# NinV/Background-Debiased-Video-CIL

Hardware: AMD Instinct MI355X
Metric: clips/sec fwd+bwd TSM-R50 8x224^2 bs32/GPU (higher is better)
Workload: dtype f32; 1 GPU; TSM-ResNet50 fwd+bwd+SGD step, synthetic 32x8x3x224x224 clips per GPU, 101 classes, SimpleLinear+CrossEntropyLoss, dropout 0.5, random-init weights; fp32 tensors, accumulators and results; conv products: fp32 via 3xbf16 split, 6 MFMA products, fp32 accumulate (dropped terms <= 2^-24 relative); conv_arith=bf16x3, clips_per_gpu=32, global_batch=32, parallelism=dp1

## Files before the change

background-debiased-video-cil_amd/_lib.py:

```python
from __future__ import annotations

import ctypes
import os
from ctypes import POINTER, Structure, c_char_p, c_float, c_int, c_int32, c_int64, c_size_t, c_uint16, c_uint64, c_void_p

_HERE = os.path.dirname(os.path.abspath(__file__))
_OVERRIDE = os.environ.get('BDVCIL_LIB_PATH')
LIB_PATH = _OVERRIDE or os.path.join(_HERE, 'csrc', 'libbdvcil_hip.so')
ABI_VERSION = 32

_lib = None


class ConvGeom(Structure):
    _fields_ = [(n, c_int32) for n in
                ('N', 'H', 'W', 'Cin', 'Ho', 'Wo', 'Cout', 'R', 'S', 'stride', 'pad', 'T', 'fold', 'pad_w', 'Rt', 'st_t', 'act_dtype')]

    def key(self):
        return tuple(getattr(self, n) for n, _ in self._fields_)


P = c_void_p
_F3 = c_float * 3

# ... 74 lines not shown
    'bdv_avgpool_fwd': (c_int, [P, P, c_int, c_int, c_int, c_int, P]),
    'bdv_avgpool_bwd': (c_int, [P, P, c_int, c_int, c_int, c_int, P]),
    'bdv_bgmix_normalize_u8': (c_int, [P, P, c_int, P, c_float, _F3, _F3, _F3, P, P, c_int, c_int, c_int, c_int, P]),
    'bdv_bg_resize_crop_u8': (c_int, [P, c_int, c_int, c_int, c_int, c_int, P, P, c_int, c_int, P, P]),
    'bdv_resize_linear_u8': (c_int, [P, c_int, c_int, c_int, P, c_int, P, P, c_int, c_int, P]),
    'bdv_jpeg_parse': (c_int, [P, c_size_t, POINTER(JpegInfo)]),
    'bdv_jpeg_entropy_decode': (c_int, [P, c_size_t, POINTER(JpegInfo), P]),
    'bdv_jpeg_entropy_decode_batch': (c_int, [P, P, c_int, POINTER(JpegInfo), P, P, c_int]),
    'bdv_jpeg_workspace_bytes': (c_size_t, [POINTER(JpegInfo), c_int]),
    'bdv_jpeg_reconstruct_u8': (c_int, [P, P, POINTER(JpegInfo), c_int, P, c_size_t, P, P]),
    'bdv_temporal_median_u8': (c_int, [P, c_int64, P, P, P, P, c_int, c_int, c_int, P, P]),
    'bdv_jpeg_encode_info': (c_int, [c_int, c_int, c_int, POINTER(JpegInfo)]),
    'bdv_jpeg_forward_u8': (c_int, [P, c_int, c_int, c_int, c_int, P, P]),
    'bdv_jpeg_encode_bound': (c_size_t, [c_int, c_int]),
    'bdv_jpeg_entropy_encode': (c_int, [P, c_int, c_int, c_int, P, c_size_t, P]),
    'bdv_jpeg_entropy_encode_batch': (c_int, [P, c_int, c_int, c_int, c_int, P, c_size_t, P, c_int]),
    'bdv_crop_normalize_u8': (c_int, [P, P, c_int, c_int, c_int, _F3, _F3, P, P, c_int, c_int, c_int, c_int, P]),
    'bdv_actor_cut_mix_u8': (c_int, [P, c_int, c_int, c_int, P, c_int, c_int, c_int, P, P, c_int64, c_int, c_int, c_int, c_int, _F3, _F3, P,
                                     c_int, P, P]),
    'bdv_lsc_fwd': (c_int, [P, P, P, P, P, P, c_int, c_int, c_int, c_int, P]),
    'bdv_lsc_bwd': (c_int, [P, P, P, P, P, P, P, P, c_float, P, c_int, c_int, c_int, c_int, P]),
    'bdv_linear_fwd': (c_int, [P, P, P, P, c_int, c_int, c_int, P]),
    'bdv_linear_bwd': (c_int, [P, P, P, P, P, P, c_float, c_int, c_int, c_int, P]),
    'bdv_consensus_fwd': (c_int, [P, P, c_int, c_int, c_int, P]),
    'bdv_consensus_bwd': (c_int, [P, P, c_int, c_int, c_int, P]),
    'bdv_dropout': (c_int, [P, P, c_int64, c_float, c_uint64, P]),
    'bdv_lsc_loss': (c_int, [P, P, P, c_float, c_int, P, P, P, P, c_int, c_int, P]),
    'bdv_softce_loss': (c_int, [P, P, P, P, P, c_int, c_int, P]),
    'bdv_icarl_targets': (c_int, [P, P, c_int, P, P, c_int, c_int, P]),
    'bdv_acm_targets': (c_int, [P, P, P, c_float, P, c_int, c_int, P]),
    'bdv_softmax_mean': (c_int, [P, P, c_int, c_int, c_int, c_int, P]),
    'bdv_topk_acc': (c_int, [P, P, P, c_int, c_int, P]),
    'bdv_repr_from_features': (c_int, [P, P, P, c_int, c_int, c_int, c_int, P]),
    'bdv_nme_workspace_bytes': (c_size_t, [c_int, c_int]),
    'bdv_nme_classify': (c_int, [P, P, P, P, c_int, c_int, c_int, c_int, P, c_size_t, P]),
    'bdv_class_means': (c_int, [P, P, P, c_int, c_int, c_int, P]),
    'bdv_herding_workspace_bytes': (c_size_t, [c_int, c_int]),
    'bdv_herding_select': (c_int, [P, c_int, c_int, c_int, c_int, P, P, P, P, c_size_t, P]),
    'bdv_randaug_workspace_bytes': (c_size_t, [c_int, c_int, c_int, c_int]),
    'bdv_randaug_apply': (c_int, [P, P, P, P, c_int, c_int, c_int, c_int, P, c_size_t, P]),
    'bdv_reduce_workspace_bytes': (c_size_t, []),
    'bdv_kd_mse_fwd': (c_int, [P, P, P, c_int64, P, c_size_t, c_int, P]),
    'bdv_kd_mse_bwd': (c_int, [P, P, P, c_float, P, c_int64, c_int, P]),
    'bdv_multi_sqnorm': (c_int, [P, P, c_int, P, P, c_size_t, P]),
    'bdv_clip_coef': (c_int, [P, c_float, c_float, P, P]),
    'bdv_multi_sgd': (c_int, [P, P, P, P, P, P, c_int, c_float, c_float, P, P]),
}


class HipExtensionError(RuntimeError):
    pass


HASHED_SOURCES = ('conv_mfma.hip', 'bn.hip', 'pool_frontend.hip', 'head_loss.hip', 'repr.hip', 'augment.hip', 'optim.hip', 'jpeg.hip',
                  'background.hip', 'actor_cut_mix.hip', 'api_common.cpp', 'common.h', 'resize_linear.h', 'Makefile', '../../include/bdvcil_hip.h')


def source_hash():
    import hashlib
    h = hashlib.sha256()
    base = os.path.join(_HERE, 'csrc')
    for name in HASHED_SOURCES:
        path = os.path.join(base, name)
        if not os.path.exists(path):
            return None
        with open(path, 'rb') as f:
            h.update(f.read())
    return h.hexdigest()


def lib():
    global _lib
    if _lib is None:
        if not os.path.exists(LIB_PATH):
            raise HipExtensionError(
                f'HIP extension not built: {LIB_PATH} is missing. Run `python -c "import __graft_entry__ as g; '
                f'g.build()"` (or `make -C {os.path.dirname(LIB_PATH)}`). There is no CPU fallback.')
        handle = ctypes.CDLL(LIB_PATH)
        for name, (res, args) in SIGNATURES.items():
            fn = getattr(handle, name)
            fn.restype = res
            fn.argtypes = args
        if handle.bdv_abi_version() != ABI_VERSION:
            raise HipExtensionError(f'ABI mismatch: library {handle.bdv_abi_version()} != binding {ABI_VERSION}')
        want, have = source_hash(), handle.bdv_source_hash().decode()
        if want is not None and want != have and not _OVERRIDE:
            raise HipExtensionError(f'stale library: {LIB_PATH} was built from other sources (hash {have[:12]}, in-tree '
                                    f'{want[:12]}). Rebuild: make -C {os.path.dirname(LIB_PATH)}')
        _lib = handle
    return _lib


def check(code: int, what: str = ''):
    if code != 0:
        msg = lib().bdv_last_error()
        raise HipExtensionError(f'{what or "bdvcil_hip"} failed with code {code}: {msg.decode() if msg else ""}')
```

background-debiased-video-cil_amd/csrc/conv_mfma.hip:

```cpp
#include <stdlib.h>
#include "common.h"

#ifdef BDV_STAMPS
__device__ unsigned long long* g_stamp_buf = nullptr;
__device__ int g_stamp_cap = 0;
#define BDV_STAMP(slot)                                                                                                          \
  do {                                                                                                                           \
    if (threadIdx.x == 0 && g_stamp_buf != nullptr && (int)(blockIdx.x + gridDim.x * blockIdx.y) < g_stamp_cap) {                 \
      unsigned long long* q_ = g_stamp_buf + (size_t)(blockIdx.x + gridDim.x * blockIdx.y) * 8;                                  \
      if ((slot) == 4) asm volatile("s_waitcnt vmcnt(0)" ::: "memory");                                                          \
      q_[slot] = __builtin_amdgcn_s_memtime();                                                                                   \
      if ((slot) == 0) { q_[5] = __builtin_amdgcn_s_memrealtime(); q_[7] = __builtin_amdgcn_s_getreg((4 << 0) | (0 << 6) | (31 << 11)); } \
      if ((slot) == 4) q_[6] = __builtin_amdgcn_s_memrealtime();                                                                 \
    }                                                                                                                            \
  } while (0)
#else
#define BDV_STAMP(slot) do { } while (0)
#endif

namespace {

constexpr int BK = 32;

struct Geom {
  int N, H, W, Cin, Ho, Wo, Cout, R, S, stride, pad, pad_w, T, fold;
  int Rt, st_t;
  float rcp_RS, rcp_S;
  int M;
  int Ktot;
  float rcp_HoWo, rcp_Wo;
  int stagger;
};

typedef unsigned int u32x4 __attribute__((ext_vector_type(4)));
constexpr int kOOB = (int)0x80000000;

__device__ __forceinline__ float4 buf_load16(__amdgpu_buffer_rsrc_t rsrc, int voff, int soff) {
  const u32x4 v = __builtin_amdgcn_raw_buffer_load_b128(rsrc, voff, soff, 0);
  return make_float4(__uint_as_float(v.x), __uint_as_float(v.y), __uint_as_float(v.z), __uint_as_float(v.w));
}

__device__ __forceinline__ void buf_store16(__amdgpu_buffer_rsrc_t rsrc, int voff, float4 v) {
  u32x4 d;
  d.x = __float_as_uint(v.x);
  d.y = __float_as_uint(v.y);
  d.z = __float_as_uint(v.z);
  d.w = __float_as_uint(v.w);
  __builtin_amdgcn_raw_buffer_store_b128(d, rsrc, voff, 0, 0);
}

typedef unsigned int u32x2v __attribute__((ext_vector_type(2)));
template <int ES>
__device__ __forceinline__ float4 buf_ld4(__amdgpu_buffer_rsrc_t rsrc, int voff) {
  if constexpr (ES == 4) {
    return buf_load16(rsrc, voff, 0);
  } else {
    const u32x2v v = __builtin_amdgcn_raw_buffer_load_b64(rsrc, voff, 0, 0);
    return bdv_widen_bf16x4(v.x, v.y);
  }
}
template <int ES>
__device__ __forceinline__ void buf_st4(__amdgpu_buffer_rsrc_t rsrc, int voff, float4 v) {
  if constexpr (ES == 4) {
    buf_store16(rsrc, voff, v);
  } else {
    __builtin_amdgcn_raw_buffer_store_b64((u32x2v){bdv_pack_bf16x2(v.x, v.y), bdv_pack_bf16x2(v.z, v.w)}, rsrc, voff, 0, 0);
  }
}

__device__ __forceinline__ void fast_divmod(int m, int d, float rcp, int& q, int& r) {
  q = (int)((float)m * rcp);
  r = m - q * d;
  if (r < 0) {
    r += d;
    --q;
  }
  if (r >= d) {
    r -= d;
    ++q;
  }
}

template <int LDA, int LDB, int TM, int TN, int MS, int NS, bool SWA, bool SWB>
__device__ __forceinline__ void mma_stage(const float* __restrict__ As, const float* __restrict__ Bs,
                                          f32x16 (&acc)[TM][TN], int wm0, int wn0, int lane) {
  const int r = lane & 31, h = lane >> 5;
  const float* apv[SWA ? 8 : 1];
  const float* bpv[SWB ? 8 : 1];
#pragma unroll
  for (int c = 0; c < (SWA ? 8 : 1); ++c) apv[c] = As + h * LDA + wm0 + (r ^ (4 * c));
#pragma unroll
  for (int c = 0; c < (SWB ? 8 : 1); ++c) bpv[c] = Bs + h * LDB + wn0 + (r ^ (4 * c));
  auto ap = [&](int s, int i) { return apv[SWA ? ((s >> 1) & 7) : 0][2 * s * LDA + MS * i]; };
  auto bp = [&](int s, int j) { return bpv[SWB ? ((s >> 1) & 7) : 0][2 * s * LDB + NS * j]; };
  float a[2][TM], b[2][TN];
#pragma unroll
  for (int i = 0; i < TM; ++i) a[0][i] = ap(0, i);
#pragma unroll
  for (int j = 0; j < TN; ++j) b[0][j] = bp(0, j);
#pragma unroll
  for (int s = 0; s < BK / 2; ++s) {
    const int cur = s & 1, nxt = cur ^ 1;
    if (s + 1 < BK / 2) {
#pragma unroll
      for (int i = 0; i < TM; ++i) a[nxt][i] = ap(s + 1, i);
#pragma unroll
      for (int j = 0; j < TN; ++j) b[nxt][j] = bp(s + 1, j);
    }
#pragma unroll
    for (int i = 0; i < TM; ++i)
#pragma unroll
      for (int j = 0; j < TN; ++j)
        acc[i][j] = __builtin_amdgcn_mfma_f32_32x32x2f32(a[cur][i], b[cur][j], acc[i][j], 0, 0, 0);
    __builtin_amdgcn_sched_group_barrier(0x100, TM + TN, 0);
    __builtin_amdgcn_sched_group_barrier(0x008, TM * TN, 0);
  }
}

__device__ __forceinline__ int shift_class(int c, int fold) {
  return (fold > 0) ? (c < fold ? 1 : (c < 2 * fold ? -1 : 0)) : 0;
}

template <int LD, int PASSES>
__device__ __forceinline__ void store_transposed(float* __restrict__ dst, const float4 (&v)[PASSES], int tid) {
  const int row = tid >> 3, kg = tid & 7;
#pragma unroll
  for (int p = 0; p < PASSES; ++p) {
    float* d = dst + (4 * kg) * LD + ((row + 32 * p) ^ (4 * kg));
    d[0] = v[p].x;
    d[LD] = v[p].y;
    d[2 * LD] = v[p].z;
    d[3 * LD] = v[p].w;
  }
}

template <int LD, int COLS, int PASSES>
__device__ __forceinline__ void store_direct(float* __restrict__ dst, const float4 (&v)[PASSES], int tid) {
  constexpr int V = COLS / 4;
#pragma unroll
  for (int p = 0; p < PASSES; ++p) {
    const int idx = tid + 256 * p;
    const int krow = idx / V, c4 = idx - krow * V;
    *reinterpret_cast<float4*>(dst + krow * LD + 4 * c4) = v[p];
  }
}

__device__ __forceinline__ int acc_row(int reg, int lane) { return (reg & 3) + 8 * (reg >> 2) + 4 * (lane >> 5); }

struct Work {
  int dp_tiles, rem_tiles, split;
};

__device__ __forceinline__ int xcd_remap(int b, int n) {
  const int q = n >> 3, r = n & 7, x = b & 7, j = b >> 3;
  return (x < r ? x * (q + 1) : r * (q + 1) + (x - r) * q) + j;
}

struct WorkItem {
  int tile, kb, ke, pslot;
};

__device__ __forceinline__ WorkItem get_work(int b, const Work& wk, int nk) {
  WorkItem it;
  if (b < wk.dp_tiles) {
    it.tile = xcd_remap(b, wk.dp_tiles);
    it.kb = 0;
    it.ke = nk;
    it.pslot = -1;
  } else {
    const int rem = b - wk.dp_tiles;
    const int rt = rem / wk.split, sl = rem - rt * wk.split;
    it.tile = wk.dp_tiles + rt;
    it.kb = (int)(((long long)sl * nk) / wk.split);
    it.ke = (int)(((long long)(sl + 1) * nk) / wk.split);
    it.pslot = wk.split > 1 ? rem : -1;
  }
  return it;
}

template <int TM, int TN, int NT = 256>
__device__ __forceinline__ void store_partial(float* __restrict__ slab, int pslot, const f32x16 (&acc)[TM][TN], int tid) {
  float* base = slab + (size_t)pslot * (TM * TN * 16) * NT + tid;
#pragma unroll
  for (int i = 0; i < TM; ++i)
#pragma unroll
    for (int j = 0; j < TN; ++j)
#pragma unroll
      for (int e = 0; e < 16; ++e) base[(size_t)((i * TN + j) * 16 + e) * NT] = acc[i][j][e];
}

template <int TM, int TN>
__device__ __forceinline__ void zero_acc(f32x16 (&acc)[TM][TN]) {
#pragma unroll
  for (int i = 0; i < TM; ++i)
#pragma unroll
    for (int j = 0; j < TN; ++j)
#pragma unroll
      for (int e = 0; e < 16; ++e) acc[i][j][e] = 0.f;
}

// ... 372 lines not shown
#pragma unroll
  for (int p = 0; p < BP; ++p) b_base[p] = ((nt * BN + arow + 32 * p) * g.Ktot + 4 * kg) * 4;

  const int RS = g.R * g.S;
  int chunk = it.kb / RS, r, s;
  {
    const int tap = it.kb - chunk * RS;
    r = tap / g.S;
    s = tap - r * g.S;
  }

  float4 ra[AP], rb[BP];
  auto load = [&]() {
    const int cls = shift_class(chunk * BK + 4 * kg, g.fold);
    const int koff_a = ((r * g.W + s) * g.Cin + chunk * BK) * 4;
    const int koff_b = ((r * g.S + s) * g.Cin + chunk * BK) * 4;
#pragma unroll
    for (int p = 0; p < AP; ++p) {
      const bool v = (unsigned)(a_hi0[p] + r) < (unsigned)g.H && (unsigned)(a_wi0[p] + s) < (unsigned)g.W &&
                     (unsigned)(a_t[p] + cls) < (unsigned)g.T;
      ra[p] = buf_load16(xr, (a_base[p] + koff_a + cls * frame_bytes) | (v ? 0 : kOOB), 0);
    }
#pragma unroll
    for (int p = 0; p < BP; ++p) rb[p] = buf_load16(wr, b_base[p], koff_b);
    s += 1;
    const int ws_ = (s == g.S) ? 1 : 0;
    s = ws_ ? 0 : s;
    r += ws_;
    const int wr_ = (r == g.R) ? 1 : 0;
    r = wr_ ? 0 : r;
    chunk += wr_;
  };

  f32x16 acc[TM][TN];
  zero_acc<TM, TN>(acc);

  load();
  for (int kt = it.kb; kt < it.ke; ++kt) {
    __syncthreads();
    store_transposed<LDA, AP>(As, ra, tid);
    store_transposed<LDB, BP>(Bs, rb, tid);
    __syncthreads();
    if (kt + 1 < it.ke) load();
    mma_stage<LDA, LDB, TM, TN, 32 * WM, 32 * WN, true, true>(As, Bs, acc, wm0, wn0, lane);
  }

  if (it.pslot >= 0) {
    store_partial<TM, TN>(slab, it.pslot, acc, tid);
    return;
  }
  fprop_epilogue<BM, BN, WM, WN>(acc, smem, y, g, epi, mt, nt, tid);
}

typedef __bf16 bf16x8_t __attribute__((ext_vector_type(8)));
typedef __bf16 bf16x4_t __attribute__((ext_vector_type(4)));
typedef float f32x4_t __attribute__((ext_vector_type(4)));
constexpr int X3_LDK = BK + 8;

typedef __bf16 bf16x2_t __attribute__((ext_vector_type(2)));
typedef float f32x2_t __attribute__((ext_vector_type(2)));
typedef unsigned u32x2_t __attribute__((ext_vector_type(2)));
__device__ __forceinline__ unsigned pack_bf16x2(float a, float b) {
  return __builtin_bit_cast(unsigned, __builtin_convertvector((f32x2_t){a, b}, bf16x2_t));
}
__device__ __forceinline__ u32x2_t bf16_hi_pairs(const float4 v) { return (u32x2_t){pack_bf16x2(v.x, v.y), pack_bf16x2(v.z, v.w)}; }
__device__ __forceinline__ void split3_pairs(const float4 v, u32x2_t& hi, u32x2_t& mid, u32x2_t& lo) {
  const unsigned h0 = pack_bf16x2(v.x, v.y), h1 = pack_bf16x2(v.z, v.w);
  const float rx = v.x - __uint_as_float(h0 << 16), ry = v.y - __uint_as_float(h0 & 0xffff0000u);
  const float rz = v.z - __uint_as_float(h1 << 16), rw = v.w - __uint_as_float(h1 & 0xffff0000u);
  const unsigned m0 = pack_bf16x2(rx, ry), m1 = pack_bf16x2(rz, rw);
  const float sx = rx - __uint_as_float(m0 << 16), sy = ry - __uint_as_float(m0 & 0xffff0000u);
  const float sz = rz - __uint_as_float(m1 << 16), sw = rw - __uint_as_float(m1 & 0xffff0000u);
  hi = (u32x2_t){h0, h1};
  mid = (u32x2_t){m0, m1};
  lo = (u32x2_t){pack_bf16x2(sx, sy), pack_bf16x2(sz, sw)};
}

template <int ROWS, int P>
__device__ __forceinline__ void store_split3(unsigned short* __restrict__ dst, const float4 (&v)[P], int tid) {
  const int arow = tid >> 3, kg = tid & 7;
#pragma unroll
  for (int p = 0; p < P; ++p) {
    u32x2_t hi, mid, lo;
    split3_pairs(v[p], hi, mid, lo);
    unsigned short* q = dst + (arow + 32 * p) * X3_LDK + 4 * kg;
    *reinterpret_cast<u32x2_t*>(q) = hi;
    *reinterpret_cast<u32x2_t*>(q + ROWS * X3_LDK) = mid;
    *reinterpret_cast<u32x2_t*>(q + 2 * ROWS * X3_LDK) = lo;
  }
}

template <int TM, int TN, int MS, int NS, int ROWS_A, int ROWS_B>
__device__ __forceinline__ void mma_stage_x3(const unsigned short* __restrict__ As, const unsigned short* __restrict__ Bs,
                                             f32x16 (&acc)[TM][TN], int wm0, int wn0, int lane) {
  const int r = lane & 31, h = lane >> 5;
#pragma unroll
  for (int s = 0; s < BK / 16; ++s) {
    bf16x8_t a[3][TM], b[3][TN];
#pragma unroll
    for (int p = 0; p < 3; ++p) {
#pragma unroll
      for (int i = 0; i < TM; ++i)
        a[p][i] = *reinterpret_cast<const bf16x8_t*>(As + (p * ROWS_A + wm0 + MS * i + r) * X3_LDK + 16 * s + 8 * h);
#pragma unroll
      for (int j = 0; j < TN; ++j)
        b[p][j] = *reinterpret_cast<const bf16x8_t*>(Bs + (p * ROWS_B + wn0 + NS * j + r) * X3_LDK + 16 * s + 8 * h);
    }
#pragma unroll
    for (int i = 0; i < TM; ++i)
#pragma unroll
      for (int j = 0; j < TN; ++j) {
        acc[i][j] = __builtin_amdgcn_mfma_f32_32x32x16_bf16(a[1][i], b[1][j], acc[i][j], 0, 0, 0);
        acc[i][j] = __builtin_amdgcn_mfma_f32_32x32x16_bf16(a[0][i], b[2][j], acc[i][j], 0, 0, 0);
        acc[i][j] = __builtin_amdgcn_mfma_f32_32x32x16_bf16(a[2][i], b[0][j], acc[i][j], 0, 0, 0);
        acc[i][j] = __builtin_amdgcn_mfma_f32_32x32x16_bf16(a[0][i], b[1][j], acc[i][j], 0, 0, 0);
        acc[i][j] = __builtin_amdgcn_mfma_f32_32x32x16_bf16(a[1][i], b[0][j], acc[i][j], 0, 0, 0);
        acc[i][j] = __builtin_amdgcn_mfma_f32_32x32x16_bf16(a[0][i], b[0][j], acc[i][j], 0, 0, 0);
      }
  }
}

template <int BM, int BN, int WM, int WN, bool BPRE = false>
__global__ __launch_bounds__(256, 2) void conv_fprop_x3_kernel(const float* __restrict__ x, const float* __restrict__ w,
                                                          float* __restrict__ y, Geom g, int NT, Work wk,
                                                          float* __restrict__ slab, FpropEpi epi) {
  constexpr int TM = BM / WM / 32, TN = BN / WN / 32;
  constexpr int AP = BM / 32, BP = BN / 32;
  static_assert(3 * (BM + BN) * X3_LDK * 2 >= WM * 32 * BN * 4, "the epilogue stages a tile pass in the same LDS");
  __shared__ __attribute__((aligned(16))) unsigned short smem16[3 * (BM + BN) * X3_LDK];
// ... 1955 lines not shown
  if (ncols % 256 != 0) return taps > 1 && stride == 1 ? 1 : (small_tiles && taps == 1 && stride == 1 && nk >= 16 ? 4 : -1);
  if (stride == 2 && taps > 1) return 0;
  if (small_tiles && shifted && taps == 1) return 4;
  if (nk <= 8 && ncols >= 1024) return -1;
  if (shifted && taps == 1 && (ncols >= 512 || nk >= 4)) return -1;
  if (ncols == 512 && nk >= 64) return 0;
  return 2;
}

PlPlan plan_pl(int cfg, int M, int ncols, int nk, size_t ws_bytes, bool ksplit_ok) {
  PlPlan p;
  p.cfg = cfg;
  p.est_us = 0.0;
  if (cfg < 0) return p;
  const PlCfg& k = kPlCfg[cfg];
  p.MT = (M + k.BM - 1) / k.BM;
  p.NT = ncols / k.BN;
  p.nk = nk;
  p.seg_bytes = (size_t)k.BM * k.BN * sizeof(float);
  if (ksplit_ok && cfg != 4) {
    p.wk = plan_work_pl(p.MT * p.NT, nk, k.iter_us, p.seg_bytes, ws_bytes, &p.est_us, pl_cfg_round(cfg));
  } else {
    p.wk.dp_tiles = p.MT * p.NT;
    p.wk.rem_tiles = 0;
    p.wk.split = 1;
    p.est_us = (double)((p.MT * p.NT + 255) / 256) * nk * k.iter_us;
  }
  return p;
}

constexpr bool r1_planes_enabled() { return true; }

bool c4_x3_enabled() {
  static const bool on = getenv("BDVCIL_C4_X3") == nullptr || atoi(getenv("BDVCIL_C4_X3")) != 0;
  return on;
}

int pl_fprop_cfg(const bdv_conv_geom* g, int pieces = 3) {
  if (g->Cin % BK != 0) return -1;
  return pl_pick(false, g->Cout, g->R * g->S * g->Cin / BK, g->R * g->S, g->stride, pieces);
}
int pl_dgrad_cfg(const bdv_conv_geom* g, int pieces = 3) {
  if (g->Cout % BK != 0) return -1;
  return pl_pick(true, g->Cin, g->R * g->S * g->Cout / BK, g->R * g->S, g->stride, pieces, g->fold > 0);
}
bool pl_fprop_ok(const bdv_conv_geom* g, int pieces = 3) { return pl_fprop_cfg(g, pieces) >= 0; }
int pl_fprop_cfg_pre(const bdv_conv_geom* g) {
  if (g->Cin % BK != 0 || g->Cout % 64 != 0) return -1;
  const int cfg = pl_fprop_cfg(g, 3);
  if (cfg >= 0) return cfg;
  return g->Cout % 256 == 0 ? 0 : g->Cout % 128 == 0 ? 1 : 3;
}
bool pl_dgrad_ok(const bdv_conv_geom* g, int pieces = 3) { return pl_dgrad_cfg(g, pieces) >= 0; }


struct WgradPlan {
  bool small;
  bool c4;
  int MTw, NTw, splits, kt_per_split;
};

WgradPlan plan_wgrad(const bdv_conv_geom* g) {
  static const int W = getenv("BDVCIL_WGRAD_W") ? atoi(getenv("BDVCIL_WGRAD_W")) : 768;
  WgradPlan p;
  p.c4 = (g->Cin % BK) != 0;
  p.small = p.c4 || (g->Cout % 128) != 0 || (g->Cin % 128) != 0;
  const int bm = p.small ? 64 : 128, bn = p.small ? 64 : 128;
  const int ktot = g->R * g->S * g->Cin;
  p.MTw = g->Cout / bm;
  p.NTw = p.c4 ? (ktot + bn - 1) / bn : g->R * g->S * (g->Cin / bn);
  const int64_t M = (int64_t)g->N * g->Ho * g->Wo;
  const int nkt = (int)((M + BK - 1) / BK);
  const int tiles = p.MTw * p.NTw;
  int best_s = 1;
  double best_cost = 1e30;
  const double dw_bytes = (double)g->Cout * ktot * 4.0;
  const int Wk = p.small ? 2 * W : W;
  for (int k = 1; k <= 4; ++k) {
    int sp = (int)(((long long)k * Wk) / tiles);
    if (sp < 1) sp = 1;
    if (sp > 1024) sp = 1024;
    while (sp > 1 && (nkt + sp - 1) / sp < 4) --sp;
    const int per = (nkt + sp - 1) / sp;
    const double rounds = (double)(((long long)tiles * sp + Wk - 1) / Wk);
    const double t_iter = 1.7 * 3.0 * (p.small ? 0.25 : 1.0);
    const double cost = rounds * per * t_iter + 4.0 + sp * dw_bytes / 4.0e6;
    if (cost < best_cost) {
      best_cost = cost;
      best_s = sp;
    }
  }
  const int per = (nkt + best_s - 1) / best_s;
  p.kt_per_split = per;
  p.splits = (nkt + per - 1) / per;
  return p;
}

bool wgrad_two_stage() {
  const char* e = getenv("BDVCIL_WGRAD_2STAGE");
  return e == nullptr || atoi(e) != 0;
}

int pl_wgrad_form(const bdv_conv_geom* g) {
  static const bool small_on = getenv("BDVCIL_PL_WGRAD64") == nullptr || atoi(getenv("BDVCIL_PL_WGRAD64")) != 0;
  const int RS = g->R * g->S;
  if (g->Cin % 128 == 0 && g->Cout % 128 == 0) return 0;
// ... 227 lines not shown
  BDV_LAUNCH_CHECK("bdv_conv_dgrad");
  if (p.wk.split > 1) {
    const dim3 fg(p.wk.rem_tiles);
    if (p.wide)
      hipLaunchKernelGGL((conv_dgrad_fixup_kernel<128, 128, 2, 2>), fg, dim3(256), 0, s, (const float*)slab, dx, add_src, add_mask_src, g, p.NT, p.wk, stat);
    else
      hipLaunchKernelGGL((conv_dgrad_fixup_kernel<128, 64, 2, 2>), fg, dim3(256), 0, s, (const float*)slab, dx, add_src, add_mask_src, g, p.NT, p.wk, stat);
    BDV_LAUNCH_CHECK("bdv_conv_dgrad(fixup)");
  }
  return BDV_OK;
}
}

extern "C" int bdv_conv_dgrad(const float* dy, const float* w, float* dx, const float* add_src,
                              const uint32_t* add_mask_src, const bdv_conv_geom* gg, const bdv_bn_stat_fuse* bn_stat,
                              void* workspace, size_t workspace_bytes, void* stream) {
  return conv_dgrad_impl(dy, w, nullptr, dx, add_src, add_mask_src, gg, bn_stat, workspace, workspace_bytes, stream);
}

extern "C" int bdv_conv_dgrad_x3(const float* dy, const float* w, const float* w_t, float* dx, const float* add_src,
                                 const uint32_t* add_mask_src, const bdv_conv_geom* gg, const bdv_bn_stat_fuse* bn_stat,
                                 void* workspace, size_t workspace_bytes, void* stream) {
  BDV_REQUIRE(w_t != nullptr, "bdv_conv_dgrad_x3: w_t is null");
  return conv_dgrad_impl(dy, w, w_t, dx, add_src, add_mask_src, gg, bn_stat, workspace, workspace_bytes, stream);
}

extern "C" size_t bdv_conv_weight_planes_bytes(const bdv_conv_geom* gg) {
  if (check_geom(gg, "bdv_conv_weight_planes_bytes")) return 0;
  return (size_t)3 * gg->Cout * gg->R * gg->S * gg->Cin * sizeof(unsigned short);
}

#ifdef BDV_STAMPS
extern "C" int bdv_debug_set_stamps(void* buf, int cap_workgroups) {
  unsigned long long* p = (unsigned long long*)buf;
  if (hipMemcpyToSymbol(HIP_SYMBOL(g_stamp_buf), &p, sizeof(p)) != hipSuccess) return -1;
  if (hipMemcpyToSymbol(HIP_SYMBOL(g_stamp_cap), &cap_workgroups, sizeof(int)) != hipSuccess) return -1;
  return 0;
}
#endif

extern "C" int bdv_conv_debug_force_tile(int cfg) {
  BDV_REQUIRE(cfg >= -1 && cfg <= kNumPlCfg, "bdv_conv_debug_force_tile: cfg %d (-1 automatic, 0 = 128x256, 1 = 256x128, 2 = 256x256, 3 = 256x64, 4 = 64x128 (dgrad), 5 = 128x128 (four waves), 6 = none)", cfg);
  g_pl_tile_forced = cfg;
  return BDV_OK;
}

extern "C" int bdv_conv_kernel_name(const bdv_conv_geom* gg, int kind, int arith, char* out, size_t n) {
  if (int e = check_geom(gg, "bdv_conv_kernel_name")) return e;
  BDV_REQUIRE(out && n > 0 && kind >= 0 && kind <= 2, "bdv_conv_kernel_name: bad argument");
  const bool c4 = gg->Cin % BK != 0;
  const int pieces = arith == 2 ? 1 : arith == 3 ? 2 : 3;
  if (kind == 0) {
    const int cfg = arith ? pl_fprop_cfg(gg, pieces) : -1;
    if (cfg >= 0) {
      snprintf(out, n, "conv_fprop_pl_kernel<%d, %d, %d, %d, %d, %d>", kPlCfg[cfg].BM, kPlCfg[cfg].BN, pl_cfg_wm(cfg), pl_cfg_wn(cfg), kPlCfg[cfg].nbuf, pieces);
    } else if (c4) {
      snprintf(out, n, "conv_fprop_c4_%skernel<128, %d, 2, 2>", arith && c4_x3_enabled() ? "x3_" : "", gg->Cout % 128 == 0 ? 128 : 64);
    } else if (gg->Cout % 128 == 0 && arith) {
      snprintf(out, n, "conv_fprop_x3_kernel<128, 128, 2, 2, %s>", r1_planes_enabled() ? "true" : "false");
    } else {
      snprintf(out, n, "conv_fprop_kernel<128, %d, 2, 2>", gg->Cout % 128 == 0 ? 128 : 64);
    }
  } else if (kind == 1) {
    const int cfg = arith ? pl_dgrad_cfg(gg, pieces) : -1;
    if (cfg >= 0) {
      snprintf(out, n, "conv_dgrad_pl_kernel<%d, %d, %d, %d, %d, %d>", kPlCfg[cfg].BM, kPlCfg[cfg].BN, pl_cfg_wm(cfg), pl_cfg_wn(cfg), kPlCfg[cfg].nbuf, pieces);
    } else if (gg->Cin % 128 == 0 && arith) {
      snprintf(out, n, "conv_dgrad_x3_kernel<128, 128, 2, 2, %s>", r1_planes_enabled() ? "true" : "false");
    } else {
      snprintf(out, n, "conv_dgrad_kernel<128, %d, 2, 2>", gg->Cin % 128 == 0 ? 128 : 64);
    }
  } else {
    if (arith && pl_wgrad_ok(gg)) {
      const WgradPlPlan p = plan_wgrad_pl(gg);
      snprintf(out, n, "conv_wgrad_pl_kernel<%d, %d", p.BM, p.BN);
    } else {
      const WgradPlan p = plan_wgrad(gg);
      snprintf(out, n, "conv_wgrad_kernel<%d, %d, 2, 2", p.small ? 64 : 128, p.small ? 64 : 128);
    }
  }
  return BDV_OK;
}

extern "C" int bdv_conv_uses_planes(const bdv_conv_geom* gg, int kind, int pieces) {
  if (check_geom(gg, "bdv_conv_uses_planes")) return 0;
  if (kind == 0) return pl_fprop_ok(gg, pieces) || (pieces >= 2 && r1_planes_enabled() && gg->Cin % BK == 0 && gg->Cout % 128 == 0) ? 1 : 0;
  if (kind == 1) return pl_dgrad_ok(gg, pieces) || (pieces >= 2 && r1_planes_enabled() && gg->Cout % BK == 0 && gg->Cin % 128 == 0) ? 1 : 0;
  return 0;
}

extern "C" int bdv_conv_fprop_pl_stat_rows(const bdv_conv_geom* gg, int pieces) {
  if (check_geom(gg, "bdv_conv_fprop_pl_stat_rows")) return 0;
  if (!pl_fprop_ok(gg, pieces)) return bdv_conv_fprop_stat_rows(gg);
  const PlPlan p = plan_pl(pl_fprop_cfg(gg, pieces), gg->N * gg->Ho * gg->Wo, gg->Cout, gg->R * gg->S * gg->Cin / BK, kMaxSplitWorkspace, true);
  return p.cfg >= 0 ? p.MT : 0;
}

extern "C" int bdv_conv_fprop_pre_stat_rows(const bdv_conv_geom* gg) {
  if (check_geom(gg, "bdv_conv_fprop_pre_stat_rows")) return 0;
  const int cfg = pl_fprop_cfg_pre(gg);
  if (cfg < 0) return 0;
  const PlPlan p = plan_pl(cfg, gg->N * gg->Ho * gg->Wo, gg->Cout, gg->R * gg->S * gg->Cin / BK, kMaxSplitWorkspace, true);
  return p.MT;
}

extern "C" int bdv_conv_dgrad_pl_stat_rows(const bdv_conv_geom* gg, int pieces) {
  if (check_geom(gg, "bdv_conv_dgrad_pl_stat_rows")) return 0;
  if (!pl_dgrad_ok(gg, pieces)) return bdv_conv_dgrad_stat_rows(gg);
  const int st = gg->stride;
  const int Mc0 = gg->N * ((gg->H + st - 1) / st) * ((gg->W + st - 1) / st);
  const PlPlan p = plan_pl(pl_dgrad_cfg(gg, pieces), st == 1 ? gg->N * gg->H * gg->W : Mc0, gg->Cin, gg->R * gg->S * gg->Cout / BK,
                           kMaxSplitWorkspace, st == 1);
  return p.cfg >= 0 ? st * st * p.MT : 0;
}

extern "C" int bdv_conv_split_weights(const float* w, const bdv_conv_geom* gg, void* planes_fprop, void* planes_dgrad, void* stream) {
  if (int e = check_geom(gg, "bdv_conv_split_weights")) return e;
  BDV_REQUIRE(w && (planes_fprop || planes_dgrad), "bdv_conv_split_weights: null pointer");
  BDV_REQUIRE(gg->Cin % 32 == 0 && gg->Cout % 32 == 0, "bdv_conv_split_weights: Cin=%d and Cout=%d must be multiples of 32", gg->Cin, gg->Cout);
  BDV_REQUIRE(bdv_aligned16(w) && bdv_aligned16(planes_fprop) && bdv_aligned16(planes_dgrad), "bdv_conv_split_weights: alignment");
  const dim3 grid(gg->Cin / 32, gg->Cout / 32, gg->R * gg->S);
  hipLaunchKernelGGL(split_weights_kernel, grid, dim3(256), 0, (hipStream_t)stream, w, (unsigned short*)planes_fprop,
                     (unsigned short*)planes_dgrad, gg->Cout, gg->R * gg->S, gg->Cin);
  BDV_LAUNCH_CHECK("bdv_conv_split_weights");
  return BDV_OK;
}

extern "C" int bdv_conv_fprop_pre_ok(const bdv_conv_geom* gg) {
  if (check_geom(gg, "bdv_conv_fprop_pre_ok")) return 0;
  return pl_fprop_cfg_pre(gg) >= 0 && gg->fold == 0 ? 1 : 0;
}

extern "C" int bdv_conv_fprop_pl(const void* x, const float* w, const void* planes_fprop, void* y, const bdv_conv_geom* gg,
                                 float* bn_partial, const bdv_conv_affine* affine, void* workspace, size_t workspace_bytes,
                                 int pieces, const float* pre_scale, const float* pre_shift, void* stream) {
  if (int e = check_geom(gg, "bdv_conv_fprop_pl")) return e;
  BDV_REQUIRE(pieces >= 1 && pieces <= 3, "bdv_conv_fprop_pl: pieces = %d (3, 2 or 1)", pieces);
  const bool pre = pre_scale != nullptr;
  const bool h16 = gg->act_dtype == BDV_ACT_BF16;
  BDV_REQUIRE_ACT(gg->act_dtype, "bdv_conv_fprop_pl");
  if (h16)
    BDV_REQUIRE(pieces == 1 && !pre && planes_fprop != nullptr && pl_fprop_ok(gg, 1),
                "bdv_conv_fprop_pl: bf16 activation storage needs pieces = 1, the weight planes, Cin %% 32 == 0 and Cout %% 64 == 0 (Cin=%d Cout=%d)", gg->Cin, gg->Cout);
  if (pre) {
    BDV_REQUIRE(pre_shift != nullptr && planes_fprop != nullptr && pieces == 3 && gg->fold == 0 && pl_fprop_cfg_pre(gg) >= 0,
                "bdv_conv_fprop_pl: a producer BatchNorm in the loader needs the plane kernels (pieces 3, no temporal shift, Cin %% 32 == 0)");
    BDV_REQUIRE(bdv_aligned16(pre_scale) && bdv_aligned16(pre_shift), "bdv_conv_fprop_pl: pre_scale / pre_shift must be 16-byte aligned");
  }
  if (!pre && (planes_fprop == nullptr || !pl_fprop_ok(gg, pieces)))
    return conv_fprop_impl((const float*)x, w, (float*)y, gg, bn_partial, affine, workspace, workspace_bytes, stream, true,
                           gg->Cin % BK == 0 && r1_planes_enabled() ? planes_fprop : nullptr);
  BDV_REQUIRE(x && y, "bdv_conv_fprop_pl: null pointer");
  FpropEpi epi = {bn_partial, 0, nullptr, nullptr, nullptr, 0, pre_scale, pre_shift};
  if (affine != nullptr) {
    BDV_REQUIRE(bn_partial == nullptr, "bdv_conv_fprop_pl: batch statistics and the folded eval-mode BatchNorm exclude each other");
    BDV_REQUIRE(affine->scale && affine->shift, "bdv_conv_fprop_pl: null pointer in bdv_conv_affine");
    BDV_REQUIRE(bdv_aligned16(affine->scale) && bdv_aligned16(affine->shift) && bdv_aligned16(affine->residual),
                "bdv_conv_fprop_pl: bdv_conv_affine pointers must be 16-byte aligned");
    epi.scale = affine->scale;
    epi.shift = affine->shift;
    epi.res = affine->residual;
    epi.relu = affine->relu;
  }
  BDV_REQUIRE(bdv_aligned16(x) && bdv_aligned16(planes_fprop) && bdv_aligned16(y) && bdv_aligned16(workspace),
              "bdv_conv_fprop_pl: pointers must be 16-byte aligned");
  Geom g = make_geom(gg);
  g.M = g.N * g.Ho * g.Wo;
  g.Ktot = g.Rt * g.R * g.S * g.Cin;
  BDV_REQUIRE((int64_t)3 * g.Cout * g.Ktot * 2 < (1ll << 31), "bdv_conv_fprop_pl: weight planes exceed 2^31 bytes");
  hipStream_t s = (hipStream_t)stream;
  const PlPlan p = plan_pl(pre ? pl_fprop_cfg_pre(gg) : pl_fprop_cfg(gg, pieces), g.M, g.Cout, g.Ktot / BK, workspace ? (workspace_bytes < kMaxSplitWorkspace ? workspace_bytes : kMaxSplitWorkspace) : 0, !h16);
  BDV_REQUIRE(p.cfg >= 0, "bdv_conv_fprop_pl: no tile configuration for Cout=%d", g.Cout);
  const int blocks = p.wk.dp_tiles + p.wk.rem_tiles * p.wk.split;
  epi.MT = p.MT;
  float* slab = (float*)workspace;
  const unsigned short* wp = (const unsigned short*)planes_fprop;
  if (debug_plan())
    fprintf(stderr, "[bdv plan] fprop_pl %dx%d Cin %d Cout %d k%d s%d: cfg %d tiles %d nk %d -> dp %d rem %d split %d (est %.0f us)\n", g.H,
            g.W, g.Cin, g.Cout, g.R, g.stride, p.cfg, p.MT * p.NT, p.nk, p.wk.dp_tiles, p.wk.rem_tiles, p.wk.split, p.est_us);
#define BDV_FPROP_PL(BM_, BN_, WM_, WN_, NB_)                                                                                         \
  do {                                                                                                                                \
    if (h16)                                                                                                                          \
      hipLaunchKernelGGL((conv_fprop_pl_kernel<BM_, BN_, WM_, WN_, NB_, 1, false, 2>), dim3(blocks), dim3(64 * WM_ * WN_), 0, s, x, wp, y, \
                         g, p.NT, p.wk, slab, epi);                                                                                   \
    else if (pre)                                                                                                                     \
      hipLaunchKernelGGL((conv_fprop_pl_kernel<BM_, BN_, WM_, WN_, NB_, 3, true>), dim3(blocks), dim3(64 * WM_ * WN_), 0, s, x, wp, y,  \
                         g, p.NT, p.wk, slab, epi);                                                                                   \
    else if (pieces == 1)                                                                                                             \
      hipLaunchKernelGGL((conv_fprop_pl_kernel<BM_, BN_, WM_, WN_, NB_, 1>), dim3(blocks), dim3(64 * WM_ * WN_), 0, s, x, wp, y, g,    \
                         p.NT, p.wk, slab, epi);                                                                                      \
    else if (pieces == 2)                                                                                                             \
      hipLaunchKernelGGL((conv_fprop_pl_kernel<BM_, BN_, WM_, WN_, NB_, 2>), dim3(blocks), dim3(64 * WM_ * WN_), 0, s, x, wp, y, g,    \
                         p.NT, p.wk, slab, epi);                                                                                      \
    else                                                                                                                              \
      hipLaunchKernelGGL((conv_fprop_pl_kernel<BM_, BN_, WM_, WN_, NB_, 3>), dim3(blocks), dim3(64 * WM_ * WN_), 0, s, x, wp, y, g,    \
                         p.NT, p.wk, slab, epi);                                                                                      \
    BDV_LAUNCH_CHECK("bdv_conv_fprop_pl");                                                                                            \
    if (p.wk.split > 1) {                                                                                                             \
      hipLaunchKernelGGL((conv_fprop_fixup_kernel<BM_, BN_, WM_, WN_>), dim3(p.wk.rem_tiles), dim3(64 * WM_ * WN_), 0, s,             \
                         (const float*)slab, (float*)y, g, p.NT, p.wk, epi);                                                                  \
      BDV_LAUNCH_CHECK("bdv_conv_fprop_pl(fixup)");                                                                                   \
// ... 284 lines not shown
```

Baseline: 590.0 clips/s.

## Add persistent streaming 1x1 conv fprop kernel with LDS-resident split filter planes

Adds a persistent kernel for stride-1 1x1 convolutions (64->64, 64->256, 256->64) in fp32 activations. Each workgroup loads all three bf16 filter planes into LDS once. Each wave then streams 128-row tiles, staging activations per wave and splitting them into three bf16 pieces for the six-product MFMA scheme. The kernel also applies the temporal shift and writes BN partial sums in the same pass. The goal is to avoid reloading filter tiles and the tiled GEMM overhead on these memory-bound layers, at the cost of relying on LDS capacity and a fixed workgroup count capped at 256.

Result: no change. 590.3 clips/s, median of 4 (+0.1%).

```diff
diff --git a/background-debiased-video-cil_amd/_lib.py b/background-debiased-video-cil_amd/_lib.py
--- a/background-debiased-video-cil_amd/_lib.py
+++ b/background-debiased-video-cil_amd/_lib.py
@@ -150,8 +150,9 @@
     pass
 
 
-HASHED_SOURCES = ('conv_mfma.hip', 'bn.hip', 'pool_frontend.hip', 'head_loss.hip', 'repr.hip', 'augment.hip', 'optim.hip', 'jpeg.hip',
-                  'background.hip', 'actor_cut_mix.hip', 'api_common.cpp', 'common.h', 'resize_linear.h', 'Makefile', '../../include/bdvcil_hip.h')
+HASHED_SOURCES = ('conv_mfma.hip', 'conv_stream1x1.hip', 'bn.hip', 'pool_frontend.hip', 'head_loss.hip', 'repr.hip', 'augment.hip', 'optim.hip', 'jpeg.hip',
+                  'background.hip', 'actor_cut_mix.hip', 'api_common.cpp', 'common.h', 'conv_shared.h', 'conv_stream1x1.h',
+                  'resize_linear.h', 'Makefile', '../../include/bdvcil_hip.h')
 
 
 def source_hash():
diff --git a/background-debiased-video-cil_amd/csrc/conv_mfma.hip b/background-debiased-video-cil_amd/csrc/conv_mfma.hip
--- a/background-debiased-video-cil_amd/csrc/conv_mfma.hip
+++ b/background-debiased-video-cil_amd/csrc/conv_mfma.hip
@@ -1,5 +1,7 @@
 #include <stdlib.h>
 #include "common.h"
+#include "conv_shared.h"
+#include "conv_stream1x1.h"
 
 #ifdef BDV_STAMPS
 __device__ unsigned long long* g_stamp_buf = nullptr;
@@ -68,19 +70,6 @@
   }
 }
 
-__device__ __forceinline__ void fast_divmod(int m, int d, float rcp, int& q, int& r) {
-  q = (int)((float)m * rcp);
-  r = m - q * d;
-  if (r < 0) {
-    r += d;
-    --q;
-  }
-  if (r >= d) {
-    r -= d;
-    ++q;
-  }
-}
-
 template <int LDA, int LDB, int TM, int TN, int MS, int NS, bool SWA, bool SWB>
 __device__ __forceinline__ void mma_stage(const float* __restrict__ As, const float* __restrict__ Bs,
                                           f32x16 (&acc)[TM][TN], int wm0, int wn0, int lane) {
@@ -117,10 +106,6 @@
   }
 }
 
-__device__ __forceinline__ int shift_class(int c, int fold) {
-  return (fold > 0) ? (c < fold ? 1 : (c < 2 * fold ? -1 : 0)) : 0;
-}
-
 template <int LD, int PASSES>
 __device__ __forceinline__ void store_transposed(float* __restrict__ dst, const float4 (&v)[PASSES], int tid) {
   const int row = tid >> 3, kg = tid & 7;
@@ -144,8 +129,6 @@
     *reinterpret_cast<float4*>(dst + krow * LD + 4 * c4) = v[p];
   }
 }
-
-__device__ __forceinline__ int acc_row(int reg, int lane) { return (reg & 3) + 8 * (reg >> 2) + 4 * (lane >> 5); }
 
 struct Work {
   int dp_tiles, rem_tiles, split;
@@ -624,29 +607,10 @@
   fprop_epilogue<BM, BN, WM, WN>(acc, smem, y, g, epi, mt, nt, tid);
 }
 
-typedef __bf16 bf16x8_t __attribute__((ext_vector_type(8)));
 typedef __bf16 bf16x4_t __attribute__((ext_vector_type(4)));
 typedef float f32x4_t __attribute__((ext_vector_type(4)));
 constexpr int X3_LDK = BK + 8;
 
-typedef __bf16 bf16x2_t __attribute__((ext_vector_type(2)));
-typedef float f32x2_t __attribute__((ext_vector_type(2)));
-typedef unsigned u32x2_t __attribute__((ext_vector_type(2)));
-__device__ __forceinline__ unsigned pack_bf16x2(float a, float b) {
-  return __builtin_bit_cast(unsigned, __builtin_convertvector((f32x2_t){a, b}, bf16x2_t));
-}
-__device__ __forceinline__ u32x2_t bf16_hi_pairs(const float4 v) { return (u32x2_t){pack_bf16x2(v.x, v.y), pack_bf16x2(v.z, v.w)}; }
-__device__ __forceinline__ void split3_pairs(const float4 v, u32x2_t& hi, u32x2_t& mid, u32x2_t& lo) {
-  const unsigned h0 = pack_bf16x2(v.x, v.y), h1 = pack_bf16x2(v.z, v.w);
-  const float rx = v.x - __uint_as_float(h0 << 16), ry = v.y - __uint_as_float(h0 & 0xffff0000u);
-  const float rz = v.z - __uint_as_float(h1 << 16), rw = v.w - __uint_as_float(h1 & 0xffff0000u);
-  const unsigned m0 = pack_bf16x2(rx, ry), m1 = pack_bf16x2(rz, rw);
-  const float sx = rx - __uint_as_float(m0 << 16), sy = ry - __uint_as_float(m0 & 0xffff0000u);
-  const float sz = rz - __uint_as_float(m1 << 16), sw = rw - __uint_as_float(m1 & 0xffff0000u);
-  hi = (u32x2_t){h0, h1};
-  mid = (u32x2_t){m0, m1};
-  lo = (u32x2_t){pack_bf16x2(sx, sy), pack_bf16x2(sz, sw)};
-}
 
 template <int ROWS, int P>
 __device__ __forceinline__ void store_split3(unsigned short* __restrict__ dst, const float4 (&v)[P], int tid) {
@@ -2708,6 +2672,8 @@
   return g->Cout % 256 == 0 ? 0 : g->Cout % 128 == 0 ? 1 : 3;
 }
 bool pl_dgrad_ok(const bdv_conv_geom* g, int pieces = 3) { return pl_dgrad_cfg(g, pieces) >= 0; }
+
+bool stream1x1_fprop_route(const bdv_conv_geom* g, int pieces) { return pieces == 3 && pl_tile_override() < 0 && bdv_stream1x1_fprop_ok(g) != 0; }
 
 
 struct WgradPlan {
@@ -3041,7 +3007,9 @@
   const int pieces = arith == 2 ? 1 : arith == 3 ? 2 : 3;
   if (kind == 0) {
     const int cfg = arith ? pl_fprop_cfg(gg, pieces) : -1;
-    if (cfg >= 0) {
+    if (arith && stream1x1_fprop_route(gg, pieces)) {
+      bdv_stream1x1_fprop_name(gg, out, n);
+    } else if (cfg >= 0) {
       snprintf(out, n, "conv_fprop_pl_kernel<%d, %d, %d, %d, %d, %d>", kPlCfg[cfg].BM, kPlCfg[cfg].BN, pl_cfg_wm(cfg), pl_cfg_wn(cfg), kPlCfg[cfg].nbuf, pieces);
     } else if (c4) {
       snprintf(out, n, "conv_fprop_c4_%skernel<128, %d, 2, 2>", arith && c4_x3_enabled() ? "x3_" : "", gg->Cout % 128 == 0 ? 128 : 64);
@@ -3073,14 +3041,14 @@
 
 extern "C" int bdv_conv_uses_planes(const bdv_conv_geom* gg, int kind, int pieces) {
   if (check_geom(gg, "bdv_conv_uses_planes")) return 0;
-  if (kind == 0) return pl_fprop_ok(gg, pieces) || (pieces >= 2 && r1_planes_enabled() && gg->Cin % BK == 0 && gg->Cout % 128 == 0) ? 1 : 0;
+  if (kind == 0) return stream1x1_fprop_route(gg, pieces) || pl_fprop_ok(gg, pieces) || (pieces >= 2 && r1_planes_enabled() && gg->Cin % BK == 0 && gg->Cout % 128 == 0) ? 1 : 0;
   if (kind == 1) return pl_dgrad_ok(gg, pieces) || (pieces >= 2 && r1_planes_enabled() && gg->Cout % BK == 0 && gg->Cin % 128 == 0) ? 1 : 0;
   return 0;
 }
 
 extern "C" int bdv_conv_fprop_pl_stat_rows(const bdv_conv_geom* gg, int pieces) {
   if (check_geom(gg, "bdv_conv_fprop_pl_stat_rows")) return 0;
-  if (!pl_fprop_ok(gg, pieces)) return bdv_conv_fprop_stat_rows(gg);
+  if (stream1x1_fprop_route(gg, pieces) || !pl_fprop_ok(gg, pieces)) return bdv_conv_fprop_stat_rows(gg);
   const PlPlan p = plan_pl(pl_fprop_cfg(gg, pieces), gg->N * gg->Ho * gg->Wo, gg->Cout, gg->R * gg->S * gg->Cin / BK, kMaxSplitWorkspace, true);
   return p.cfg >= 0 ? p.MT : 0;
 }
@@ -3136,6 +3104,8 @@
                 "bdv_conv_fprop_pl: a producer BatchNorm in the loader needs the plane kernels (pieces 3, no temporal shift, Cin %% 32 == 0)");
     BDV_REQUIRE(bdv_aligned16(pre_scale) && bdv_aligned16(pre_shift), "bdv_conv_fprop_pl: pre_scale / pre_shift must be 16-byte aligned");
   }
+  if (!pre && !h16 && affine == nullptr && planes_fprop != nullptr && stream1x1_fprop_route(gg, pieces))
+    return bdv_stream1x1_fprop((const float*)x, planes_fprop, (float*)y, bn_partial, gg, stream);
   if (!pre && (planes_fprop == nullptr || !pl_fprop_ok(gg, pieces)))
     return conv_fprop_impl((const float*)x, w, (float*)y, gg, bn_partial, affine, workspace, workspace_bytes, stream, true,
                            gg->Cin % BK == 0 && r1_planes_enabled() ? planes_fprop : nullptr);
diff --git a/background-debiased-video-cil_amd/csrc/conv_shared.h b/background-debiased-video-cil_amd/csrc/conv_shared.h
--- /dev/null
+++ b/background-debiased-video-cil_amd/csrc/conv_shared.h
@@ -0,0 +1,42 @@
+#pragma once
+#include "common.h"
+
+typedef __bf16 bf16x8_t __attribute__((ext_vector_type(8)));
+typedef __bf16 bf16x2_t __attribute__((ext_vector_type(2)));
+typedef float f32x2_t __attribute__((ext_vector_type(2)));
+typedef unsigned u32x2_t __attribute__((ext_vector_type(2)));
+
+__device__ __forceinline__ unsigned pack_bf16x2(float a, float b) {
+  return __builtin_bit_cast(unsigned, __builtin_convertvector((f32x2_t){a, b}, bf16x2_t));
+}
+__device__ __forceinline__ u32x2_t bf16_hi_pairs(const float4 v) { return (u32x2_t){pack_bf16x2(v.x, v.y), pack_bf16x2(v.z, v.w)}; }
+__device__ __forceinline__ void split3_pairs(const float4 v, u32x2_t& hi, u32x2_t& mid, u32x2_t& lo) {
+  const unsigned h0 = pack_bf16x2(v.x, v.y), h1 = pack_bf16x2(v.z, v.w);
+  const float rx = v.x - __uint_as_float(h0 << 16), ry = v.y - __uint_as_float(h0 & 0xffff0000u);
+  const float rz = v.z - __uint_as_float(h1 << 16), rw = v.w - __uint_as_float(h1 & 0xffff0000u);
+  const unsigned m0 = pack_bf16x2(rx, ry), m1 = pack_bf16x2(rz, rw);
+  const float sx = rx - __uint_as_float(m0 << 16), sy = ry - __uint_as_float(m0 & 0xffff0000u);
+  const float sz = rz - __uint_as_float(m1 << 16), sw = rw - __uint_as_float(m1 & 0xffff0000u);
+  hi = (u32x2_t){h0, h1};
+  mid = (u32x2_t){m0, m1};
+  lo = (u32x2_t){pack_bf16x2(sx, sy), pack_bf16x2(sz, sw)};
+}
+
+__device__ __forceinline__ void fast_divmod(int m, int d, float rcp, int& q, int& r) {
+  q = (int)((float)m * rcp);
+  r = m - q * d;
+  if (r < 0) {
+    r += d;
+    --q;
+  }
+  if (r >= d) {
+    r -= d;
+    ++q;
+  }
+}
+
+__device__ __forceinline__ int shift_class(int c, int fold) {
+  return (fold > 0) ? (c < fold ? 1 : (c < 2 * fold ? -1 : 0)) : 0;
+}
+
+__device__ __forceinline__ int acc_row(int reg, int lane) { return (reg & 3) + 8 * (reg >> 2) + 4 * (lane >> 5); }
diff --git a/background-debiased-video-cil_amd/csrc/conv_stream1x1.h b/background-debiased-video-cil_amd/csrc/conv_stream1x1.h
--- /dev/null
+++ b/background-debiased-video-cil_amd/csrc/conv_stream1x1.h
@@ -0,0 +1,8 @@
+#pragma once
+#include "common.h"
+
+int bdv_stream1x1_fprop_ok(const bdv_conv_geom* g);
+
+int bdv_stream1x1_fprop(const float* x, const void* planes_fprop, float* y, float* bn_partial, const bdv_conv_geom* g, void* stream);
+
+void bdv_stream1x1_fprop_name(const bdv_conv_geom* g, char* out, size_t n);
diff --git a/background-debiased-video-cil_amd/csrc/conv_stream1x1.hip b/background-debiased-video-cil_amd/csrc/conv_stream1x1.hip
--- /dev/null
+++ b/background-debiased-video-cil_amd/csrc/conv_stream1x1.hip
@@ -0,0 +1,215 @@
+#include <stdlib.h>
+#include "common.h"
+#include "conv_shared.h"
+#include "conv_stream1x1.h"
+
+namespace {
+
+constexpr int kWaves = 8;
+constexpr int kStageBytes = 32 * 64 * 4;
+constexpr int kOOB = (int)0x80000000;
+constexpr int kCUs = 256;
+
+typedef unsigned int u32x4 __attribute__((ext_vector_type(4)));
+
+struct S1Params {
+  int M;
+  int tiles;
+  int HW;
+  int CL;
+  float rcp_CL;
+  int fold;
+};
+
+__device__ __forceinline__ void wave_lds_fence() {
+  __builtin_amdgcn_fence(__ATOMIC_ACQ_REL, "wavefront");
+  __builtin_amdgcn_wave_barrier();
+}
+
+template <int CIN, int COUT>
+__global__ __launch_bounds__(64 * kWaves, 2) void conv_stream1x1_fprop_kernel(const float* __restrict__ x,
+                                                                              const unsigned short* __restrict__ wp,
+                                                                              float* __restrict__ y, float* __restrict__ bn_partial,
+                                                                              S1Params p) {
+  constexpr int KC = CIN / 64;
+  constexpr int NT = COUT / 32;
+  constexpr int NH = NT > 4 ? NT / 4 : 1;
+  constexpr int TH = NT / NH;
+  constexpr int PB = CIN * COUT * 2;
+  static_assert(KC == 1 || NH == 1, "a strip is either one K chunk or one column pass");
+  static_assert((KC & (KC - 1)) == 0 && 3 * PB + kWaves * kStageBytes <= 160 * 1024, "filter + stages must fit the LDS");
+  __shared__ __attribute__((aligned(16))) unsigned char smem[3 * PB + kWaves * kStageBytes];
+
+  const int tid = threadIdx.x, lane = tid & 63, wave = tid >> 6;
+  for (int i = tid; i < 3 * PB / 16; i += 64 * kWaves) {
+    const int pl = i / (PB / 16), q = i - pl * (PB / 16);
+    const int row = q >> 2, c = q & 3;
+    *reinterpret_cast<u32x4*>(smem + pl * PB + row * 64 + ((c ^ ((row >> 2) & 3)) << 4)) = reinterpret_cast<const u32x4*>(wp)[i];
+  }
+  __syncthreads();
+
+  const int nwaves = gridDim.x * kWaves;
+  const int gw = wave * gridDim.x + blockIdx.x;
+  if (gw >= p.tiles) return;
+  const int units = ((p.tiles - 1 - gw) / nwaves + 1) * 4 * KC;
+
+  unsigned char* const stage = smem + 3 * PB + wave * kStageBytes;
+  const int lr = lane >> 4, lc = lane & 15;
+  const int fr = lane & 31, fh = lane >> 5;
+  const __amdgpu_buffer_rsrc_t xr = __builtin_amdgcn_make_buffer_rsrc((void*)x, 0, p.M * CIN * 4, 0x00020000);
+  const __amdgpu_buffer_rsrc_t yr = __builtin_amdgcn_make_buffer_rsrc((void*)y, 0, p.M * COUT * 4, 0x00020000);
+  const unsigned char* wb[2];
+#pragma unroll
+  for (int sp = 0; sp < 2; ++sp) wb[sp] = smem + fr * 64 + (((2 * sp + fh) ^ ((fr >> 2) & 3)) << 4);
+
+  float4 ra[8];
+  auto issue = [&](int unit) __attribute__((always_inline)) {
+    const int tile = gw + (unit / (4 * KC)) * nwaves, strip = (unit / KC) & 3, kc = unit & (KC - 1);
+    const int ch = kc * 64 + 4 * lc;
+    const int cls = shift_class(ch, p.fold);
+    const int m0 = tile * 128 + strip * 32 + lr;
+#pragma unroll
+    for (int i = 0; i < 8; ++i) {
+      const int m = m0 + 4 * i;
+      bool ok = m < p.M;
+      if (p.fold > 0) {
+        int q, pos;
+        fast_divmod(ok ? m : 0, p.CL, p.rcp_CL, q, pos);
+        ok = ok && (cls == 0 || (cls > 0 ? pos < p.CL - p.HW : pos >= p.HW));
+      }
+      const int off = ((m + cls * p.HW) * CIN + ch) * 4;
+      const u32x4 v = __builtin_amdgcn_raw_buffer_load_b128(xr, ok ? off : kOOB, 0, 0);
+      ra[i] = make_float4(__uint_as_float(v.x), __uint_as_float(v.y), __uint_as_float(v.z), __uint_as_float(v.w));
+    }
+  };
+
+  f32x16 acc[TH];
+  float cs[NT], cq[NT];
+#pragma unroll
+  for (int j = 0; j < NT; ++j) cs[j] = cq[j] = 0.f;
+
+  auto process = [&](int unit) __attribute__((always_inline)) {
+    const int tile = gw + (unit / (4 * KC)) * nwaves, strip = (unit / KC) & 3, kc = unit & (KC - 1);
+    wave_lds_fence();
+#pragma unroll
+    for (int i = 0; i < 8; ++i)
+      *reinterpret_cast<float4*>(stage + (4 * i + lr) * 256 + ((lc ^ ((4 * i + lr) & 15)) << 4)) = ra[i];
+    wave_lds_fence();
+    if (unit + 1 < units) issue(unit + 1);
+    bf16x8_t a[3][4];
+#pragma unroll
+    for (int s = 0; s < 4; ++s) {
+      const float4 v0 = *reinterpret_cast<const float4*>(stage + fr * 256 + (((4 * s + 2 * fh) ^ (fr & 15)) << 4));
+      const float4 v1 = *reinterpret_cast<const float4*>(stage + fr * 256 + (((4 * s + 2 * fh + 1) ^ (fr & 15)) << 4));
+      u32x2_t h0, m0, l0, h1, m1, l1;
+      split3_pairs(v0, h0, m0, l0);
+      split3_pairs(v1, h1, m1, l1);
+      a[0][s] = __builtin_bit_cast(bf16x8_t, (u32x4){h0.x, h0.y, h1.x, h1.y});
+      a[1][s] = __builtin_bit_cast(bf16x8_t, (u32x4){m0.x, m0.y, m1.x, m1.y});
+      a[2][s] = __builtin_bit_cast(bf16x8_t, (u32x4){l0.x, l0.y, l1.x, l1.y});
+    }
+    const int row0 = tile * 128 + strip * 32;
+#pragma unroll
+    for (int hh = 0; hh < NH; ++hh) {
+      if (kc == 0) {
+#pragma unroll
+        for (int j = 0; j < TH; ++j)
+#pragma unroll
+          for (int e = 0; e < 16; ++e) acc[j][e] = 0.f;
+      }
+#pragma unroll
+      for (int j = 0; j < TH; ++j)
+#pragma unroll
+        for (int s = 0; s < 4; ++s) {
+          const unsigned char* q = wb[s & 1] + ((2 * kc + (s >> 1)) * COUT + 32 * (hh * TH + j)) * 64;
+          const bf16x8_t b0 = *reinterpret_cast<const bf16x8_t*>(q), b1 = *reinterpret_cast<const bf16x8_t*>(q + PB),
+                         b2 = *reinterpret_cast<const bf16x8_t*>(q + 2 * PB);
+          acc[j] = __builtin_amdgcn_mfma_f32_32x32x16_bf16(a[1][s], b1, acc[j], 0, 0, 0);
+          acc[j] = __builtin_amdgcn_mfma_f32_32x32x16_bf16(a[0][s], b2, acc[j], 0, 0, 0);
+          acc[j] = __builtin_amdgcn_mfma_f32_32x32x16_bf16(a[2][s], b0, acc[j], 0, 0, 0);
+          acc[j] = __builtin_amdgcn_mfma_f32_32x32x16_bf16(a[0][s], b1, acc[j], 0, 0, 0);
+          acc[j] = __builtin_amdgcn_mfma_f32_32x32x16_bf16(a[1][s], b0, acc[j], 0, 0, 0);
+          acc[j] = __builtin_amdgcn_mfma_f32_32x32x16_bf16(a[0][s], b0, acc[j], 0, 0, 0);
+        }
+      if (kc == KC - 1) {
+        const int lane_off = ((row0 + 4 * fh) * COUT + 32 * hh * TH + fr) * 4;
+#pragma unroll
+        for (int j = 0; j < TH; ++j)
+#pragma unroll
+          for (int e = 0; e < 16; ++e) {
+            const int rr = (e & 3) + 8 * (e >> 2);
+            const float v = acc[j][e];
+            const bool ok = row0 + 4 * fh + rr < p.M;
+            __builtin_amdgcn_raw_buffer_store_b32(__float_as_uint(v), yr, ok ? lane_off + (rr * COUT + 32 * j) * 4 : kOOB, 0, 0);
+            cs[hh * TH + j] += v;
+            cq[hh * TH + j] += v * v;
+          }
+      }
+    }
+    if (strip == 3 && kc == KC - 1) {
+      if (bn_partial != nullptr) {
+#pragma unroll
+        for (int j = 0; j < NT; ++j) {
+          const float s1 = cs[j] + __shfl_xor(cs[j], 32, 64), s2 = cq[j] + __shfl_xor(cq[j], 32, 64);
+          if (fh == 0) {
+            bn_partial[(size_t)tile * COUT + 32 * j + fr] = s1;
+            bn_partial[((size_t)p.tiles + tile) * COUT + 32 * j + fr] = s2;
+          }
+        }
+      }
+#pragma unroll
+      for (int j = 0; j < NT; ++j) cs[j] = cq[j] = 0.f;
+    }
+  };
+  issue(0);
+  for (int unit = 0; unit < units; ++unit) process(unit);
+}
+
+bool stream1x1_enabled() {
+  const char* e = getenv("BDVCIL_STREAM_1X1");
+  return e == nullptr || atoi(e) != 0;
+}
+
+int stream1x1_workgroups(int tiles) {
+  int wgs = (tiles + kWaves - 1) / kWaves;
+  if (wgs > kCUs) wgs = kCUs;
+  const char* e = getenv("BDVCIL_STREAM_1X1_WGS");
+  if (e != nullptr && atoi(e) > 0 && atoi(e) < wgs) wgs = atoi(e);
+  return wgs < 1 ? 1 : wgs;
+}
+
+}
+
+int bdv_stream1x1_fprop_ok(const bdv_conv_geom* g) {
+  if (!stream1x1_enabled()) return 0;
+  if (g->act_dtype != BDV_ACT_F32 || g->R != 1 || g->S != 1 || g->stride != 1 || g->pad != 0 || g->pad_w > 0 || g->Rt > 1) return 0;
+  return (g->Cin == 64 && (g->Cout == 64 || g->Cout == 256)) || (g->Cin == 256 && g->Cout == 64) ? 1 : 0;
+}
+
+void bdv_stream1x1_fprop_name(const bdv_conv_geom* g, char* out, size_t n) {
+  snprintf(out, n, "conv_stream1x1_fprop_kernel<%d, %d>", g->Cin, g->Cout);
+}
+
+int bdv_stream1x1_fprop(const float* x, const void* planes_fprop, float* y, float* bn_partial, const bdv_conv_geom* g, void* stream) {
+  BDV_REQUIRE(bdv_stream1x1_fprop_ok(g), "bdv_stream1x1_fprop: geometry not covered (Cin=%d Cout=%d)", g->Cin, g->Cout);
+  BDV_REQUIRE(x && planes_fprop && y, "bdv_stream1x1_fprop: null pointer");
+  BDV_REQUIRE(bdv_aligned16(x) && bdv_aligned16(planes_fprop) && bdv_aligned16(y), "bdv_stream1x1_fprop: pointers must be 16-byte aligned");
+  S1Params p;
+  p.M = g->N * g->H * g->W;
+  p.tiles = (p.M + 127) / 128;
+  p.HW = g->H * g->W;
+  p.fold = g->fold;
+  p.CL = (g->fold > 0 ? g->T : 1) * p.HW;
+  p.rcp_CL = 1.0f / (float)p.CL;
+  const dim3 grid(stream1x1_workgroups(p.tiles)), block(64 * kWaves);
+  hipStream_t s = (hipStream_t)stream;
+  const unsigned short* wp = (const unsigned short*)planes_fprop;
+  if (g->Cin == 64 && g->Cout == 256)
+    hipLaunchKernelGGL((conv_stream1x1_fprop_kernel<64, 256>), grid, block, 0, s, x, wp, y, bn_partial, p);
+  else if (g->Cin == 256)
+    hipLaunchKernelGGL((conv_stream1x1_fprop_kernel<256, 64>), grid, block, 0, s, x, wp, y, bn_partial, p);
+  else
+    hipLaunchKernelGGL((conv_stream1x1_fprop_kernel<64, 64>), grid, block, 0, s, x, wp, y, bn_partial, p);
+  BDV_LAUNCH_CHECK("bdv_stream1x1_fprop");
+  return BDV_OK;
+}
```
